# zipnn/zipnn

Hardware: NVIDIA H100
Metric: compress+decompress GB/s on bf16 tensors (higher is better)
Workload: dtype u8

## Files before the change

### zipnn_b200/csrc/decode.cuh

```cuda
#pragma once
#include <cuda.h>
#include "common.cuh"

#ifndef ZB_CPASYNC_L2
#define ZB_CPASYNC_L2 ".L2::128B"
#endif

#ifndef ZB_SIDE_SLOTS
#ifndef ZB_FUSED_MIN_BLOCKS
#define ZB_FUSED_MIN_BLOCKS 16
#endif
#define ZB_SIDE_SLOTS 4
#endif

namespace zb {

struct ItemTable;

enum : uint32_t { kModePlain = 0, kModeFused = 1, kModeGeneral = 2, kModeSkip = 3, kModeOverflow = 4 };
constexpr uint32_t kOverflowCtas = 32;
constexpr uint32_t kFillBytes = 64;

struct DecodeCfg {
  const uint8_t* body;
  uint8_t* out;
  uint64_t body_len;
  int G;
  uint64_t K;
  uint32_t chunk;
  uint64_t orig;
  int bits_mode;
  Ctrl* ctrl;
  ItemDesc* items;
  uint8_t* mode;
  uint32_t* slot;
  uint32_t* rlist;
  uint8_t* fill;
  uint8_t* planes;
  uint64_t pstride;
  uint32_t max_slots;
  uint32_t ovf_slots;
  uint32_t* olist;
  uint32_t* hlist;
  struct ItemTable* tables;
  uint32_t tma_flags;
  uint64_t k_full;
  uint64_t side_pred[3];
  uint32_t side_r0[3];
  uint64_t box_base, box_rows, box_pitch, box_len;
  uint64_t box_step_rows, box_step_cols;
  uint32_t box_fast;
  uint64_t c0;
};

constexpr uint32_t kBoxStep = 4096;

__device__ __forceinline__ bool box_meets(const DecodeCfg& cfg, uint64_t a, uint64_t n) {
  const uint64_t e0 = cfg.box_base + cfg.box_len;
  const uint64_t r = a < e0 ? 0 : (a - e0) / cfg.box_pitch + 1;
  return r < cfg.box_rows && cfg.box_base + r * cfg.box_pitch < a + n;
}
struct BoxCursor {
  int64_t row;
  uint64_t col;
};
__device__ __forceinline__ BoxCursor box_cursor(const DecodeCfg& cfg, uint64_t v) {
  BoxCursor k;
  if (v >= cfg.box_base) {
    const uint64_t q = (v - cfg.box_base) / cfg.box_pitch;
    k.row = (int64_t)q;
    k.col = v - cfg.box_base - q * cfg.box_pitch;
  } else {
    const uint64_t d = cfg.box_base - v, q = (d + cfg.box_pitch - 1) / cfg.box_pitch;
    k.row = -(int64_t)q;
    k.col = q * cfg.box_pitch - d;
  }
  return k;
}
__device__ __forceinline__ void box_advance(const DecodeCfg& cfg, BoxCursor& k) {
  k.row += (int64_t)cfg.box_step_rows;
  k.col += cfg.box_step_cols;
  if (k.col >= cfg.box_pitch) {
    k.col -= cfg.box_pitch;
    k.row++;
  }
}
__device__ __forceinline__ void box_store16(const DecodeCfg& cfg, uint8_t* __restrict__ out, const BoxCursor& k, const uint32_t (&r)[4]) {
  if (cfg.box_fast) {
    if (k.row >= 0 && (uint64_t)k.row < cfg.box_rows && k.col < cfg.box_len)
      *reinterpret_cast<uint4*>(out + (uint64_t)k.row * cfg.box_len + k.col) = make_uint4(r[0], r[1], r[2], r[3]);
    return;
  }
  int64_t row = k.row;
  uint64_t col = k.col;
#pragma unroll
  for (int i = 0; i < 16; i++) {
    if (row >= 0 && (uint64_t)row < cfg.box_rows && col < cfg.box_len) out[(uint64_t)row * cfg.box_len + col] = (uint8_t)(r[i >> 2] >> (8 * (i & 3)));
    if (++col == cfg.box_pitch) {
// ... 594 lines not shown
  bool active = false;
  uint64_t c = 0;
  int g = 0;
  if (item < nitems) {
    g = (int)(item / cfg.K);
    c = item - (uint64_t)g * cfg.K;
    if (cfg.mode[c] == kModeGeneral) {
      d = cfg.items[item];
      active = (d.kind == kHuf);
    }
  }
  if (__ballot_sync(0xffffffffu, active) == 0) return;
  planar_decode_item(S, cfg, d, active, slot, stream, active ? cfg.planes + ((uint64_t)cfg.slot[c] * cfg.G + g) * cfg.pstride : nullptr);
}

struct alignas(64) TmaMaps {
  CUtensorMap out;
  CUtensorMap side[3];
};
enum : uint32_t { kTmaOut = 1u, kTmaSide = 2u };

__device__ __forceinline__ void mbar_init(uint32_t bar_s, uint32_t count) {
  asm volatile("mbarrier.init.shared::cta.b64 [%0], %1;" ::"r"(bar_s), "r"(count) : "memory");
}
__device__ __forceinline__ void mbar_expect_tx(uint32_t bar_s, uint32_t bytes) {
  asm volatile("mbarrier.arrive.expect_tx.shared::cta.b64 _, [%0], %1;" ::"r"(bar_s), "r"(bytes) : "memory");
}
__device__ __forceinline__ void mbar_wait(uint32_t bar_s, uint32_t parity) {
  asm volatile(
      "{\n.reg .pred p;\nW_%=:\nmbarrier.try_wait.parity.shared::cta.b64 p, [%0], %1;\n@p bra D_%=;\nbra W_%=;\nD_%=:\n}\n" ::"r"(bar_s), "r"(parity)
      : "memory");
}
__device__ __forceinline__ void tma_load_2d(uint32_t dst_s, const CUtensorMap* map, uint32_t x, uint32_t y, uint32_t bar_s) {
  asm volatile("cp.async.bulk.tensor.2d.shared::cluster.global.mbarrier::complete_tx::bytes [%0], [%1, {%2, %3}], [%4];" ::"r"(dst_s),
               "l"((uint64_t)(uintptr_t)map), "r"(x), "r"(y), "r"(bar_s)
               : "memory");
}
__device__ __forceinline__ void tma_store_2d(const CUtensorMap* map, uint32_t src_s, uint32_t x, uint32_t y) {
  asm volatile("cp.async.bulk.tensor.2d.global.shared::cta.bulk_group [%0, {%2, %3}], [%1];" ::"l"((uint64_t)(uintptr_t)map), "r"(src_s), "r"(x), "r"(y)
               : "memory");
  asm volatile("cp.async.bulk.commit_group;" ::: "memory");
}
__device__ __forceinline__ void tma_store_wait_read() { asm volatile("cp.async.bulk.wait_group.read 0;" ::: "memory"); }
__device__ __forceinline__ void tma_store_wait_all() { asm volatile("cp.async.bulk.wait_group 0;" ::: "memory"); }
__device__ __forceinline__ void fence_proxy_async() { asm volatile("fence.proxy.async.shared::cta;" ::: "memory"); }

template <int G>
struct FusedGeom {
  static constexpr int kIters = 8 / G;
  static constexpr int NS = (G > 1) ? G - 1 : 1;
  static constexpr uint32_t kSlotBytes = 512u * ZB_SIDE_SLOTS;
  static constexpr int kTileIters = 2;
  static constexpr uint32_t kTileRow = 16u * kTileIters + 16u, kTileBytes = 32u * kTileRow;
  static constexpr uint32_t kTileRegion = (G == 2) ? 2u * kTileBytes : 0u;
  static constexpr uint32_t kSlotRegion = (G == 1) ? 0u : (uint32_t)(G - 1) * kSlotBytes;
  static constexpr uint32_t kSideAll = kSlotRegion > kTileRegion ? kSlotRegion : kTileRegion;
};
__host__ __device__ constexpr uint32_t fused_tail_bytes(int pb) { return pb == 0 ? 4096u : 2048u; }
__host__ __device__ constexpr uint32_t fused_tail_cap(int pb) { return fused_tail_bytes(pb) / 2u; }
template <int G>
__host__ __device__ constexpr size_t fused_smem_bytes(int pb) {
  return (pb == 0 ? (size_t)4096 + 32 * kRingBytes : (size_t)3072 + 16 * kRingBytes) + FusedGeom<G>::kSideAll + fused_tail_bytes(pb) + 32 * 128 + 16;
}
struct FusedSmem {
  unsigned char* raw;
  uint32_t base_s;
  uint32_t table_off;
  uint32_t ring_lo_off, ring_hi_off;
  uint32_t tail_off, bar_off, stage_off, side_off;
  __device__ __forceinline__ uint16_t* tail() const { return reinterpret_cast<uint16_t*>(raw + tail_off); }
  __device__ __forceinline__ uint8_t* ring(int lane) const { return raw + (lane < 16 ? ring_lo_off : ring_hi_off) + kRingBytes * (uint32_t)(lane & 15); }
  __device__ __forceinline__ uint8_t* weights(int slot) const { return raw + (slot < 4 ? ring_lo_off : ring_hi_off) + 256u * (uint32_t)(slot & 3); }
  __device__ __forceinline__ uint8_t (*stage() const)[128] { return reinterpret_cast<uint8_t (*)[128]>(raw + stage_off); }
};
template <int G, int PB>
__device__ __forceinline__ FusedSmem fused_smem_carve(unsigned char* raw) {
  FusedSmem S;
  S.raw = raw;
  S.base_s = (uint32_t)__cvta_generic_to_shared(raw);
  asm volatile("" : "+r"(S.base_s));
  uint32_t at;
  if (PB == 0) {
    S.table_off = 0;
    at = 4096;
  } else {
    S.table_off = (2048u - (S.base_s & 2047u)) & 2047u;
    S.ring_lo_off = S.table_off ? 0u : 2048u;
    at = 3072;
  }
  S.tail_off = at;
  at += fused_tail_bytes(PB);
  if (PB == 0) {
    S.ring_lo_off = at;
    at += 16 * kRingBytes;
  }
  S.ring_hi_off = at;
  at += 16 * kRingBytes;
  S.stage_off = at;
  at += 32 * 128;
  S.side_off = at;
  S.bar_off = at + FusedGeom<G>::kSideAll;
  return S;
}
template <int G>
__device__ __forceinline__ uint32_t side_tile_s(const FusedSmem& S, uint32_t st) { return S.base_s + S.side_off + st * FusedGeom<G>::kTileBytes; }
template <int G>
__device__ __forceinline__ uint32_t side_slots_s(const FusedSmem& S, int g) { return S.base_s + S.side_off + (uint32_t)g * FusedGeom<G>::kSlotBytes; }
static_assert(sizeof(FseDecSmall) <= 512, "small tANS scratch must fit in 4 stage rows");

struct SidePlane {
  const uint4* blk;
  uint32_t shift;
  uint32_t step;
  uint4 a, b;
  uint32_t slots_s;
  uint32_t swz;
};

__device__ __forceinline__ uint4 lds_u128(uint32_t saddr) {
  uint4 v;
  asm volatile("ld.shared.v4.u32 {%0, %1, %2, %3}, [%4];" : "=r"(v.x), "=r"(v.y), "=r"(v.z), "=r"(v.w) : "r"(saddr));
  return v;
}
constexpr uint32_t kSideSlots = ZB_SIDE_SLOTS;
__device__ __forceinline__ uint32_t side_slot(const SidePlane& sp, uint32_t j) { return sp.slots_s + (((j & (kSideSlots - 1u)) ^ sp.swz) << 4); }

__device__ __forceinline__ uint4 ldg128(const uint4* p) { return __ldg(p); }
__device__ __forceinline__ void take16(const uint4& a, const uint4& b, uint32_t shift, uint32_t (&out)[4]) {
  const uint32_t w[8] = {a.x, a.y, a.z, a.w, b.x, b.y, b.z, b.w};
  const uint32_t bs = (shift & 3) * 8;
  uint32_t t[7];
#pragma unroll
  for (int i = 0; i < 7; i++) t[i] = __funnelshift_r(w[i], w[i + 1], bs);
  const bool s4 = shift & 4, s8 = shift & 8;
  uint32_t u[5];
#pragma unroll
  for (int i = 0; i < 5; i++) u[i] = s8 ? t[i + 2] : t[i];
#pragma unroll
  for (int i = 0; i < 4; i++) out[i] = s4 ? u[i + 1] : u[i];
}

template <int W>
__device__ __forceinline__ void take16_w(const uint4& a, const uint4& b, uint32_t bit_shift, uint32_t (&out)[4]) {
  const uint32_t w[8] = {a.x, a.y, a.z, a.w, b.x, b.y, b.z, b.w};
#pragma unroll
  for (int i = 0; i < 4; i++) out[i] = __funnelshift_r(w[i + W], w[i + W + 1], bit_shift);
}

__device__ __forceinline__ uint32_t bitselect(uint32_t a, uint32_t b, uint32_t m) {
  uint32_t d;
  asm("lop3.b32 %0, %1, %2, %3, 0xE4;" : "=r"(d) : "r"(a), "r"(b), "r"(m));
  return d;
}
__device__ __forceinline__ void unrotate_planes_pre(uint32_t& lo, uint32_t& hi, uint32_t m) {
  const uint32_t sm = lo, e = hi;
  hi = bitselect(sm, e, m);
  lo = bitselect(e, sm, m);
}

__device__ __forceinline__ uint4* stage_unit(uint8_t (*stage)[128], int row, int unit) {
  return reinterpret_cast<uint4*>(&stage[row][((unit ^ row) & 7) * 16]);
}

template <int G>
__device__ __forceinline__ void emit_elements(uint32_t (&pl)[G][4], uint32_t rot_mask, uint8_t (*stage)[128], int lane, int unit0) {
  if (G == 1) {
    *stage_unit(stage, lane, unit0) = make_uint4(pl[0][0], pl[0][1], pl[0][2], pl[0][3]);
    return;
  }
#pragma unroll
  for (int q = 0; q < 4; q++) unrotate_planes_pre(pl[(G - 2) % G][q], pl[G - 1][q], rot_mask);
  uint32_t w[4 * G];
  if (G == 2) {
#pragma unroll
    for (int q = 0; q < 4; q++) {
      w[2 * q] = __byte_perm(pl[0][q], pl[1 % G][q], 0x5140);
      w[2 * q + 1] = __byte_perm(pl[0][q], pl[1 % G][q], 0x7362);
    }
  } else {
#pragma unroll
    for (int q = 0; q < 4; q++) {
      const uint32_t t0 = __byte_perm(pl[0][q], pl[1 % G][q], 0x5140), t1 = __byte_perm(pl[2 % G][q], pl[3 % G][q], 0x5140);
      const uint32_t t2 = __byte_perm(pl[0][q], pl[1 % G][q], 0x7362), t3 = __byte_perm(pl[2 % G][q], pl[3 % G][q], 0x7362);
      w[4 * q] = __byte_perm(t0, t1, 0x5410);
      w[4 * q + 1] = __byte_perm(t0, t1, 0x7632);
      w[4 * q + 2] = __byte_perm(t2, t3, 0x5410);
      w[4 * q + 3] = __byte_perm(t2, t3, 0x7632);
    }
  }
#pragma unroll
  for (int q = 0; q < G; q++) *stage_unit(stage, lane, unit0 + q) = make_uint4(w[4 * q], w[4 * q + 1], w[4 * q + 2], w[4 * q + 3]);
}

template <int G, class LUT>
__device__ __forceinline__ void fused_iteration(BitWindow& b, const LUT& lut, SidePlane (&side)[(G > 1) ? G - 1 : 1],
                                                const uint4* hi_block, bool guard, bool rot, uint8_t (*stage)[128], int lane, int unit0, uint32_t it,
                                                bool wait_store) {
  if (G > 1) {
#pragma unroll
    for (int g = 0; g < G - 1; g++) {
      const uint4* nb = side[g].blk + 3 * side[g].step;
      if (guard && side[g].step && nb > hi_block) nb = hi_block;
      cp_async16_s(side_slot(side[g], it + 3u), nb);
    }
  }
  uint32_t pl[G][4];
  decode16(b, lut, pl[G - 1]);
  if (wait_store) {
    if (lane == 0) tma_store_wait_read();
    __syncwarp();
  }
  if (G > 1) {
#pragma unroll
    for (int g = 0; g < G - 1; g++) take16(side[g].a, side[g].b, side[g].shift, pl[g]);
  }
  emit_elements<G>(pl, rot ? 0x80808080u : 0u, stage, lane, unit0);
  if (G > 1) {
#pragma unroll
    for (int g = 0; g < G - 1; g++) {
      side[g].a = side[g].b;
      side[g].b = lds_u128(side_slot(side[g], it + 2u));
      side[g].blk += side[g].step;
    }
  }
}

template <int G, int PB>
__global__ void __launch_bounds__(32, G == 4 ? 12 : ZB_FUSED_MIN_BLOCKS) k_huf_decode_fused(DecodeCfg cfg, uint8_t* __restrict__ out, const __grid_constant__ TmaMaps maps) {
  extern __shared__ __align__(1024) unsigned char smem_raw[];
  using Geo = FusedGeom<G>;
  using LUT = typename std::conditional<PB == 0, LutTwo, LutCol<(PB ? PB : 5)>>::type;
  constexpr int kIters = Geo::kIters;
  constexpr int NS = Geo::NS;
  const FusedSmem S = fused_smem_carve<G, PB>(smem_raw);
  const int lane = threadIdx.x, slot = lane >> 2, stream = lane & 3;
  const uint64_t K = cfg.K;
  const uint64_t ngroups = (K + kDecItemsPerWarp - 1) / kDecItemsPerWarp;
  if (PB != 0 && S.table_off > 1024u) {
    if (lane == 0 && blockIdx.x == 0) atomicOr(&cfg.ctrl->error, kErrUnsupported);
    return;
  }
  const uint32_t bar_s = S.base_s + S.bar_off;
  if (lane == 0) {
    mbar_init(bar_s, 1);
    mbar_init(bar_s + 8, 1);
    asm volatile("fence.mbarrier_init.release.cluster;" ::: "memory");
  }
  __syncwarp();
  uint32_t tiles_done = 0;
  bool store_pending = false;
  uint8_t (*const stage)[128] = S.stage();
  const uint32_t stage_s = S.base_s + S.stage_off;
  const bool rot = (cfg.bits_mode == 1) && (G > 1);
  const uint32_t rot_mask = rot ? 0x80808080u : 0u;
  const uint4* hi_block = reinterpret_cast<const uint4*>(((uintptr_t)(cfg.body + cfg.body_len) - 1) & ~(uintptr_t)15);

  for (uint64_t grp = blockIdx.x; grp < ngroups; grp += gridDim.x) {
    const uint64_t c = grp * kDecItemsPerWarp + slot;
    const bool active = (c < K) && cfg.mode[c] == kModeFused;
    if (__ballot_sync(0xffffffffu, active) == 0) continue;
    if (store_pending) {
      if (lane == 0) tma_store_wait_read();
      store_pending = false;
    }
    __syncwarp();

    ItemDesc d;
    d.kind = kRaw;
    d.src_off = 0;
    d.src_len = d.dec_len = 0;
    if (active) d = cfg.items[(uint64_t)(G - 1) * K + c];

    int lg = 0, hsize = -1, x_long = 0;
    uint32_t tail_at = 0;
    {
      uint8_t* weights = S.weights(slot);
      const bool builder = active && stream == 0;
      int nsym = 0;
      constexpr uint32_t kHdrSlot = 176;
      uint8_t* hdr = reinterpret_cast<uint8_t*>(S.tail()) + kHdrSlot * (uint32_t)slot;
      const uint8_t* tsrc = cfg.body + d.src_off;
      const uint32_t mis = (uint32_t)((uintptr_t)tsrc & 15u);
      if (active) {
        const uint8_t* body_end = cfg.body + cfg.body_len;
#pragma unroll
        for (int q = 0; q < 3; q++) {
          const int blk = stream + 4 * q;
          const uint8_t* g = tsrc - mis + 16 * blk;
          if (blk < (int)(kHdrSlot / 16) && g < body_end) *reinterpret_cast<uint4*>(hdr + 16 * blk) = ldg128(reinterpret_cast<const uint4*>(g));
        }
      }
      __syncwarp();
      if (builder) {
        FseDecSmall& D = *reinterpret_cast<FseDecSmall*>(&stage[4 * slot][0]);
        const uint32_t avail = kHdrSlot - mis;
        hsize = huf_read_weights(weights, &nsym, &lg, hdr + mis, d.src_len < avail ? d.src_len : avail, D);
        if (hsize >= 0) {
          x_long = PB == 0 ? lut2_tail_size(weights, nsym, lg) : lut_tail_size(weights, nsym, lg, PB, reinterpret_cast<uint16_t*>(&stage[4 * slot][0]));
          if (x_long < 0) hsize = -1;
        }
      }
      {
        const uint32_t mine = (builder && hsize >= 0) ? (uint32_t)x_long : 0u;
        uint32_t run = mine;
#pragma unroll
        for (int o = 4; o < 32; o <<= 1) {
          const uint32_t v = __shfl_up_sync(0xffffffffu, run, o);
          if (lane >= o) run += v;
        }
        tail_at = run - mine;
// ... 15 lines not shown
        nsym = __shfl_sync(0xffffffffu, nsym, lane & ~3);
        if (active && hsize >= 0)
          fill_lut_col<(PB ? PB : 5)>(reinterpret_cast<uint16_t*>(S.raw + S.table_off) + lane, S.tail() + tail_at, stream == 0, weights, nsym, lg, rot, (uint32_t)x_long,
                                      reinterpret_cast<const uint16_t*>(&stage[4 * slot][0]));
      }
      __syncwarp();
    }
    bool live = active && hsize >= 0;

    const uint8_t* p = cfg.body + d.src_off + (live ? hsize : 0);
    const uint32_t rest = live ? d.src_len - (uint32_t)hsize : 0;
    uint32_t l0 = 0, l1 = 0, l2 = 0, l3 = 0;
    if (live) {
      bool ok = rest >= 10;
      if (ok) {
        l0 = p[0] | (p[1] << 8);
        l1 = p[2] | (p[3] << 8);
        l2 = p[4] | (p[5] << 8);
        ok = l0 + l1 + l2 + 6 <= rest;
        l3 = rest - (l0 + l1 + l2 + 6);
        ok = ok && l0 && l1 && l2 && l3;
      }
      if (!ok) {
        atomicOr(&cfg.ctrl->error, kErrCorrupt);
        live = false;
      }
    }
    const uint32_t seg = d.dec_len >> 2;
    uint32_t s_off = 6, s_len = l0;
    if (stream == 1) { s_off += l0; s_len = l1; }
    if (stream == 2) { s_off += l0 + l1; s_len = l2; }
    if (stream == 3) { s_off += l0 + l1 + l2; s_len = l3; }
    const uint32_t out_off = (uint32_t)stream * seg;

    LUT lut;
    if constexpr (PB == 0) {
      lut.prim_s = S.base_s + S.table_off + 512u * (uint32_t)slot;
    } else {
      lut.col_s = S.base_s + S.table_off + 2u * (uint32_t)lane;
    }
    lut.tail_s = S.base_s + S.tail_off + 2u * tail_at;
    lut.hi_mask = 0x7FFu & ~((uint32_t)x_long - 1u);

    bool regular = live && c < cfg.k_full;
    if (G > 1 && regular) {
#pragma unroll
      for (int g = 0; g < G - 1; g++) {
        const ItemDesc t = cfg.items[(uint64_t)g * K + c];
        regular = regular && t.kind == kRaw && t.src_off == cfg.side_pred[g] + c * (uint64_t)(cfg.chunk / (uint32_t)G);
      }
    }
    regular = __all_sync(0xffffffffu, regular);
    const bool out_tma = regular && (cfg.tma_flags & kTmaOut);
    const bool side_tma = (G == 2) && regular && (cfg.tma_flags & kTmaSide);

    BitWindow b;
    if (live && !window_init(b, p + s_off, s_len, cfg.body, S.ring(lane))) {
      atomicOr(&cfg.ctrl->error, kErrCorrupt);
      live = false;
    }
    if (regular && !live) {
      b.cont = 0; b.s = 53; b.qm = 0; b.next = 0; b.fetch48 = 0; b.floor64 = 0xffffffffu; b.start_bit = 0;
      b.ring = S.ring(lane);
      b.ring_s = (uint32_t)__cvta_generic_to_shared(b.ring);
      b.gsrc = cfg.body;
    }

    const uint32_t rows_full = (seg >> 4) / kIters;
    if constexpr (G == 2) {
      if (side_tma) {
        const uint32_t y0 = (uint32_t)(grp * 32u);
        constexpr int kTI = Geo::kTileIters;
        constexpr int kTilesPerRow = kIters / kTI;
        const uint32_t ntiles = rows_full * (uint32_t)kTilesPerRow;
        const uint32_t r0 = cfg.side_r0[0];
        auto issue_tile = [&](uint32_t t) {
          const uint32_t st = (tiles_done + t) & 1u;
          mbar_expect_tx(bar_s + 8u * st, Geo::kTileBytes);
          tma_load_2d(side_tile_s<G>(S, st), &maps.side[0], 16u * (uint32_t)kTI * t, y0, bar_s + 8u * st);
        };
        if (lane == 0 && ntiles) issue_tile(0);
        uint8_t* flush_ptr = out + (grp * (uint64_t)kDecItemsPerWarp) * (uint64_t)cfg.chunk + (uint64_t)((uint32_t)(lane >> 3) * seg) * G +
                             (uint32_t)(lane & 7) * 16u;
        const uint32_t chunk_b = cfg.chunk;
        const bool chunk_256k = chunk_b == 262144u;
        const uint32_t bit_shift = (r0 & 3u) * 8u;
        auto run_rows = [&](auto wtag) {
          constexpr int W = decltype(wtag)::value;
          for (uint32_t row = 0; row < rows_full; row++) {
#pragma unroll
            for (int tr = 0; tr < kTilesPerRow; tr++) {
              const uint32_t t = row * (uint32_t)kTilesPerRow + (uint32_t)tr;
              const uint32_t n = tiles_done + t;
              __syncwarp();
              if (lane == 0 && t + 1 < ntiles) issue_tile(t + 1);
              mbar_wait(bar_s + 8u * (n & 1u), (n >> 1) & 1u);
              const uint32_t my_row = side_tile_s<G>(S, n & 1u) + (uint32_t)lane * Geo::kTileRow;
              uint4 blk[kTI + 1];
#pragma unroll
              for (int q = 0; q <= kTI; q++) blk[q] = lds_u128(my_row + 16u * (uint32_t)q);
#pragma unroll
              for (int ki = 0; ki < kTI; ki++) {
                uint32_t pl[G][4];
                decode16(b, lut, pl[G - 1]);
                take16_w<W>(blk[ki], blk[ki + 1], bit_shift, pl[0]);
                emit_elements<G>(pl, rot_mask, stage, lane, (tr * kTI + ki) * G);
              }
            }
            __syncwarp();
            if (chunk_256k) {
#pragma unroll
              for (int r = 0; r < 8; r++) *reinterpret_cast<uint4*>(flush_ptr + (size_t)r * 262144u) = *stage_unit(stage, r * 4 + (lane >> 3), lane & 7);
            } else {
#pragma unroll
              for (int r = 0; r < 8; r++) *reinterpret_cast<uint4*>(flush_ptr + (size_t)r * chunk_b) = *stage_unit(stage, r * 4 + (lane >> 3), lane & 7);
            }
            flush_ptr += 128;
            __syncwarp();
          }
        };
        switch (r0 >> 2) {
          case 0: run_rows(std::integral_constant<int, 0>{}); break;
          case 1: run_rows(std::integral_constant<int, 1>{}); break;
          case 2: run_rows(std::integral_constant<int, 2>{}); break;
          default: run_rows(std::integral_constant<int, 3>{}); break;
        }
        tiles_done += ntiles;
        if (live && !window_exact(b)) atomicOr(&cfg.ctrl->error, kErrCorrupt);
        continue;
      }
    }
    SidePlane side[NS];
    if (G > 1 && live) {
#pragma unroll
      for (int g = 0; g < G - 1; g++) {
        const uint64_t i = (uint64_t)g * K + c;
        const ItemDesc t = cfg.items[i];
        const uint8_t* q;
        if (t.kind == kRle) {
          q = cfg.fill + i * kFillBytes;
          side[g].step = 0;
        } else {
          q = cfg.body + t.src_off + out_off;
          side[g].step = 1;
        }
        side[g].shift = (uint32_t)((uintptr_t)q & 15);
        side[g].blk = reinterpret_cast<const uint4*>((uintptr_t)q & ~(uintptr_t)15);
        side[g].a = ldg128(side[g].blk);
        const uint4* nb = side[g].blk + side[g].step;
        side[g].b = ldg128((side[g].step && nb > hi_block) ? hi_block : nb);
        nb += side[g].step;
        side[g].swz = kSideSlots == 2 ? (((uint32_t)lane >> 2) & 1u) : (((uint32_t)lane >> 1) & 3u);
        side[g].slots_s = side_slots_s<G>(S, g) + 16u * kSideSlots * (uint32_t)lane;
        cp_async16_s(side_slot(side[g], 2u), (side[g].step && nb > hi_block) ? hi_block : nb);
      }
      cp_async_commit();
      cp_async_wait<0>();
    }

    const uint32_t my_rows = live ? rows_full : 0;
    uint32_t max_rows = my_rows;
#pragma unroll
    for (int o = 16; o; o >>= 1) max_rows = max(max_rows, __shfl_xor_sync(0xffffffffu, max_rows, o));
    if (out_tma) {
      const uint32_t y0 = (uint32_t)(grp * 32u);
      for (uint32_t row = 0; row < max_rows; row++) {
        const bool guard = row + 2 >= my_rows;
#pragma unroll
        for (int k = 0; k < kIters; k++)
          fused_iteration<G, LUT>(b, lut, side, hi_block, guard, rot, stage, lane, k * G, row * (uint32_t)kIters + (uint32_t)k, k == 0 && store_pending);
// ... 250 lines not shown
```

### zipnn_b200/csrc/common.cuh

```cuda
#pragma once
#include <cuda_runtime.h>
#include <stdint.h>
#include "huf_serial.cuh"

namespace zb {

struct Ctrl {
  uint32_t error;
  uint32_t overflow_count;
  uint64_t base[4];
  uint64_t total_len;
  uint64_t group_total[4];
  uint32_t work_counter;
  uint32_t regroup_count;
  uint32_t huf_count;
};
static_assert(sizeof(Ctrl) <= 256, "ctrl block");
constexpr size_t kCtrlBytes = 256;

struct ItemDesc {
  uint64_t src_off;
  uint32_t src_len;
  uint32_t dec_len;
  uint32_t kind;
  uint32_t pad;
};
enum : uint32_t { kRaw = 0, kRle = 1, kHuf = 2 };

enum : uint32_t { kErrCorrupt = 1u, kErrUnsupported = 2u, kErrWorkspace = 4u };

__host__ __device__ __forceinline__ uint32_t rot16(uint32_t u) {
  return ((u >> 8) & 0x00800080u) | ((u << 1) & 0xFF00FF00u) | (u & 0x007F007Fu);
}
__host__ __device__ __forceinline__ uint32_t unrot16(uint32_t u) {
  return ((u << 8) & 0x80008000u) | ((u >> 1) & 0x7F807F80u) | (u & 0x007F007Fu);
}
__host__ __device__ __forceinline__ uint32_t rot32(uint32_t u) {
  return ((u >> 8) & 0x00800000u) | ((u << 1) & 0xFF000000u) | (u & 0x007FFFFFu);
}
__host__ __device__ __forceinline__ uint32_t unrot32(uint32_t u) {
  return ((u << 8) & 0x80000000u) | ((u >> 1) & 0x7F800000u) | (u & 0x007FFFFFu);
}
template <int G>
__host__ __device__ __forceinline__ uint32_t rot_word(uint32_t u) {
  return G == 2 ? rot16(u) : (G == 4 ? rot32(u) : u);
}
template <int G>
__host__ __device__ __forceinline__ uint32_t unrot_word(uint32_t u) {
  return G == 2 ? unrot16(u) : (G == 4 ? unrot32(u) : u);
}

__host__ __device__ __forceinline__ uint32_t plane_len(uint32_t chunk_len, int G, int g) {
  return chunk_len / (uint32_t)G + ((uint32_t)g < chunk_len % (uint32_t)G ? 1u : 0u);
}

__device__ __forceinline__ uint32_t batch_find(const uint64_t* start, uint32_t n, uint64_t w) {
  uint32_t lo = 0, hi = n;
  while (hi - lo > 1) {
    const uint32_t mid = (lo + hi) >> 1;
    if (start[mid] <= w) lo = mid; else hi = mid;
  }
  return lo;
}

__device__ __forceinline__ uint64_t ld_u64_bytes(const uint8_t* p) {
  uint64_t v = 0;
#pragma unroll
  for (int i = 0; i < 8; i++) v |= (uint64_t)p[i] << (8 * i);
// ... 23 lines not shown
```

### zipnn_b200/csrc/zipnn_b200.cu

```cuda
#include "../../include/zipnn_b200.h"

#include <cuda.h>
#include <cuda_runtime.h>
#include <atomic>
#include <cstdio>
#include <cstdlib>
#include <cstring>
#include <mutex>
#include <numeric>
#include <vector>

#include "common.cuh"
#include "decode.cuh"
#include "decode_sync.cuh"
#include "encode.cuh"
#include "stage1.cuh"

using namespace zb;

namespace {

std::atomic<int> g_last_cuda_error{0};
std::atomic<unsigned long long> g_launches{0};

// ... 47 lines not shown
      a = take_event();
      cudaEventRecord(a, st);
    }
  }
  ~ScopedTimer() {
    if (a) {
      std::lock_guard<std::mutex> lk(g_timing_mu);
      cudaEvent_t b = take_event();
      cudaEventRecord(b, st);
      g_spans.push_back({id, a, b});
    }
  }
};

int sm_count_cached() {
  static int cached = 0;
  if (cached == 0) {
    int dev = 0, n = 0;
    if (cudaGetDevice(&dev) == cudaSuccess &&
        cudaDeviceGetAttribute(&n, cudaDevAttrMultiProcessorCount, dev) == cudaSuccess && n > 0)
      cached = n;
    else
      return 132;
  }
  return cached;
}

typedef CUresult (*EncodeTiledFn)(CUtensorMap*, CUtensorMapDataType, cuuint32_t, void*, const cuuint64_t*, const cuuint64_t*,
                                  const cuuint32_t*, const cuuint32_t*, CUtensorMapInterleave, CUtensorMapSwizzle,
                                  CUtensorMapL2promotion, CUtensorMapFloatOOBfill);
EncodeTiledFn tensor_map_encoder() {
  static EncodeTiledFn fn = [] {
    void* p = nullptr;
    cudaDriverEntryPointQueryResult q;
    if (cudaGetDriverEntryPoint("cuTensorMapEncodeTiled", &p, cudaEnableDefault, &q) != cudaSuccess || q != cudaDriverEntryPointSuccess) p = nullptr;
    (void)cudaGetLastError();
    return (EncodeTiledFn)p;
  }();
  return fn;
}
bool byte_map_2d(CUtensorMap* m, const void* base, uint64_t inner, uint64_t rows, uint64_t pitch, uint32_t box_inner, CUtensorMapSwizzle sw,
                 CUtensorMapL2promotion l2) {
  EncodeTiledFn enc = tensor_map_encoder();
  if (!enc || ((uintptr_t)base & 15) || (pitch & 15) || inner == 0 || rows == 0 || inner > 0xffffffffull || rows > 0xffffffffull) return false;
  cuuint64_t dims[2] = {inner, rows};
  cuuint64_t strides[1] = {pitch};
  cuuint32_t box[2] = {box_inner, 32};
  cuuint32_t es[2] = {1, 1};
  return enc(m, CU_TENSOR_MAP_DATA_TYPE_UINT8, 2, const_cast<void*>(base), dims, strides, box, es, CU_TENSOR_MAP_INTERLEAVE_NONE, sw, l2,
             CU_TENSOR_MAP_FLOAT_OOB_FILL_NONE) == CUDA_SUCCESS;
}

struct Knobs {
  int tma = 2, grid_mode = 1, warps_per_sm = 0;
  long long sync_max = -1;
  long long slice_piece = -1;
  size_t smem_pad = 0;
};
Knobs knobs() {
  Knobs k;
  if (const char* e = getenv("ZIPNN_B200_SLICE_PIECE_CHUNKS")) k.slice_piece = atoll(e);
  if (const char* e = getenv("ZIPNN_B200_TMA")) k.tma = atoi(e);
  if (const char* e = getenv("ZIPNN_B200_GRID_MODE")) k.grid_mode = atoi(e);
  if (const char* e = getenv("ZIPNN_B200_WARPS_PER_SM")) k.warps_per_sm = atoi(e);
  if (const char* e = getenv("ZIPNN_B200_SMEM_PAD")) k.smem_pad = (size_t)atoi(e);
  if (const char* e = getenv("ZIPNN_B200_SYNC_MAX")) k.sync_max = atoll(e);
  return k;
}

template <typename Kernel>
int resident_blocks(Kernel k, size_t smem) {
  int nb = 0;
  if (cudaOccupancyMaxActiveBlocksPerMultiprocessor(&nb, k, 32, smem) != cudaSuccess || nb < 1) nb = 1;
  return nb;
}

inline bool valid_layout(int num_buf, int bytes_mode, size_t chunk) {
  if (!(num_buf == 1 || num_buf == 2 || num_buf == 4)) return false;
  if (num_buf == 4 ? bytes_mode != 220 : bytes_mode != 10) return false;
  if (chunk == 0 || (chunk & (chunk - 1)) != 0 || chunk > (1ull << 31)) return false;
  if (chunk % (size_t)num_buf) return false;
  return true;
}

inline size_t round_up(size_t v, size_t a) { return (v + a - 1) / a * a; }
inline uint64_t num_chunks(size_t n, size_t chunk) { return (n + chunk - 1) / chunk; }

constexpr uint64_t kDefaultSlots = 64;
constexpr uint64_t kSyncTablesMaxChunks = 16384;
constexpr uint64_t kSyncDefaultMaxChunks = 3072;
struct DecWs {
  size_t items_off, mode_off, slot_off, rlist_off, olist_off, hlist_off, tables_off, fill_off, planes_off, pstride, fixed;
};
inline DecWs dec_ws_layout(size_t orig, int G, size_t chunk, uint64_t table_chunks = UINT64_MAX) {
  DecWs L;
  const uint64_t K = num_chunks(orig, chunk);
  if (table_chunks == UINT64_MAX) table_chunks = K <= kSyncTablesMaxChunks ? K : 0;
  L.items_off = kCtrlBytes;
  L.mode_off = round_up(L.items_off + sizeof(ItemDesc) * (size_t)G * K, 256);
  L.slot_off = round_up(L.mode_off + K, 256);
  L.rlist_off = round_up(L.slot_off + 4 * K, 256);
  L.olist_off = round_up(L.rlist_off + 4 * K, 256);
  L.hlist_off = round_up(L.olist_off + 4 * K, 256);
  L.tables_off = round_up(L.hlist_off + 4 * (size_t)G * K, 256);
  L.fill_off = round_up(L.tables_off + sizeof(ItemTable) * (size_t)G * table_chunks, 256);
  L.planes_off = round_up(L.fill_off + (size_t)kFillBytes * G * K, 256);
  L.pstride = round_up(chunk / (size_t)G, 16) + 16;
  L.fixed = L.planes_off + 256;
  return L;
}

template <typename F>
int dispatch_G(int G, F&& f) {
  switch (G) {
    case 1: return f(std::integral_constant<int, 1>());
    case 2: return f(std::integral_constant<int, 2>());
    default: return f(std::integral_constant<int, 4>());
  }
}

int read_ctrl_error(void* d_ws, cudaStream_t st) {
  uint32_t err = 0;
  ZB_CUDA(cudaMemcpyAsync(&err, d_ws, sizeof(uint32_t), cudaMemcpyDeviceToHost, st));
  ZB_CUDA(cudaStreamSynchronize(st));
  if (err & kErrCorrupt) return ZIPNN_B200_E_CORRUPT;
  if (err & kErrUnsupported) return ZIPNN_B200_E_UNSUPPORTED;
  if (err & kErrWorkspace) return ZIPNN_B200_E_CAPACITY;
// ... 160 lines not shown
      }
      static const int nb = [] {
        int v = 0;
        if (cudaOccupancyMaxActiveBlocksPerMultiprocessor(&v, k_huf_decode_sync<GG>, kSyncThreads, kSyncSmemBytes) != cudaSuccess || v < 1) v = 1;
        return v;
      }();
      const unsigned grid = (unsigned)std::min<uint64_t>(4 * nitems, (uint64_t)nb * sm_count_cached());
      {
        ScopedTimer tp(kKParseTables, st);
        k_parse_tables<<<(unsigned)((nitems + kParseWarps - 1) / kParseWarps), kParseWarps * 32, 0, st>>>(cfg);
        ZB_LAUNCHED();
      }
      ScopedTimer tm(kKHufDecodeSync, st);
      k_huf_decode_sync<GG><<<grid, kSyncThreads, kSyncSmemBytes, st>>>(cfg, (uint8_t*)d_out);
      ZB_LAUNCHED();
      return ZIPNN_B200_OK;
    });
    if (rc) return rc;
  } else {
    {
      const uint64_t groups = (K + kDecItemsPerWarp - 1) / kDecItemsPerWarp;
      if (groups > 0x7fffffffull) return ZIPNN_B200_E_ARG;
      const bool short_codes = (G >= 2 && bits_mode == 1);
      TmaMaps maps;
      memset(&maps, 0, sizeof(maps));
      cfg.tma_flags = 0;
      cfg.k_full = orig / chunk;
      const uint64_t last_len = orig - cfg.k_full * chunk;
      uint64_t at = 9ull * G * K;
      for (int g = 0; g < 3; g++) {
        cfg.side_pred[g] = at;
        cfg.side_r0[g] = (uint32_t)(((uintptr_t)d_body + at) & 15);
        if (g < G) at += cfg.k_full * (chunk / G) + plane_len((uint32_t)last_len, G, g);
      }
      if (cfg.k_full >= (uint64_t)kDecItemsPerWarp && chunk >= 2048 && (chunk / 4) * 4 == chunk) {
        if (byte_map_2d(&maps.out, d_out, chunk / 4, 4 * cfg.k_full, chunk / 4, 128, CU_TENSOR_MAP_SWIZZLE_128B, CU_TENSOR_MAP_L2_PROMOTION_NONE)) {
          cfg.tma_flags |= kTmaOut;
        if (G == 2) {
          const uint64_t seg = chunk / G / 4;
          const uint8_t* base = (const uint8_t*)d_body + cfg.side_pred[0] - cfg.side_r0[0];
          if (seg >= 64 && body_len >= cfg.side_pred[0] + 4 * cfg.k_full * seg &&
              byte_map_2d(&maps.side[0], base, seg + 16, 4 * cfg.k_full, seg, FusedGeom<2>::kTileRow, CU_TENSOR_MAP_SWIZZLE_NONE,
                          CU_TENSOR_MAP_L2_PROMOTION_L2_128B))
            cfg.tma_flags |= kTmaSide;
        }
        }
      }
      cfg.tma_flags &= (uint32_t)kn.tma;
      if (getenv("ZIPNN_B200_DEBUG")) fprintf(stderr, "[zipnn_b200] fused decode: K=%llu k_full=%llu tma_flags=%u side_r0=%u encoder=%p\n", (unsigned long long)K,
                                              (unsigned long long)cfg.k_full, cfg.tma_flags, cfg.side_r0[0], (void*)tensor_map_encoder());
      ScopedTimer tm(kKHufDecode, st);
      int rc = dispatch_G(G, [&](auto g) -> int {
        constexpr int GG = decltype(g)::value;
        const int sms = sm_count_cached();
        auto grid_for = [&](int nb) -> unsigned {
          if (kn.grid_mode == 1) return (unsigned)groups;
          if (kn.warps_per_sm > 0) nb = std::min(nb, kn.warps_per_sm);
          return (unsigned)std::min<uint64_t>(groups, (uint64_t)nb * sms);
        };
        if (short_codes) {
          const size_t smem = fused_smem_bytes<GG>(5) + kn.smem_pad;
          const int nb = resident_blocks(k_huf_decode_fused<GG, 5>, smem);
          k_huf_decode_fused<GG, 5><<<grid_for(nb), 32, smem, st>>>(cfg, (uint8_t*)d_out, maps);
        } else {
          const size_t smem = fused_smem_bytes<GG>(0) + kn.smem_pad;
          const int nb = resident_blocks(k_huf_decode_fused<GG, 0>, smem);
          k_huf_decode_fused<GG, 0><<<grid_for(nb), 32, smem, st>>>(cfg, (uint8_t*)d_out, maps);
        }
        ZB_LAUNCHED();
        return ZIPNN_B200_OK;
      });
      if (rc) return rc;
    }
    {
      const uint64_t warps = (nitems + kDecItemsPerWarp - 1) / kDecItemsPerWarp;
      if (warps > 0x7fffffffull) return ZIPNN_B200_E_ARG;
      ScopedTimer tm(kKHufDecodePlanar, st);
      k_huf_decode_planar<<<(unsigned)warps, 32, sizeof(DecodeSmem), st>>>(cfg);
      ZB_LAUNCHED();
    }
  }
  {
    const uint32_t tiles_per_chunk = (uint32_t)((chunk + kMergeTile - 1) / kMergeTile);
    const uint64_t ntiles = K * tiles_per_chunk;
    const int blocks = (int)std::min<uint64_t>(ntiles, (uint64_t)sm_count_cached() * 16);
    ScopedTimer tm(kKRegroup, st);
    int rc = dispatch_G(G, [&](auto g) -> int {
      k_regroup<decltype(g)::value><<<blocks, kMergeThreads, 0, st>>>(cfg, (uint8_t*)d_out);
      ZB_LAUNCHED();
      return ZIPNN_B200_OK;
    });
    if (rc) return rc;
  }
  if (cfg.ovf_slots) {
    ScopedTimer tm(kKDecodeOverflow, st);
    int rc = dispatch_G(G, [&](auto g) -> int {
      k_decode_overflow<decltype(g)::value><<<cfg.ovf_slots, kMergeThreads, sizeof(DecodeSmem), st>>>(cfg, (uint8_t*)d_out);
      ZB_LAUNCHED();
      return ZIPNN_B200_OK;
    });
    if (rc) return rc;
  }
  if (check) return read_ctrl_error(d_ws, st);
  return ZIPNN_B200_OK;
}

static size_t batch_header_bytes(int n) {
  return round_up(256 + sizeof(DecodeCfg) * (size_t)n + 3 * sizeof(uint64_t) * ((size_t)n + 1), 256);
}
static size_t batch_slice_bytes(const zipnn_b200_batch_item& it) {
  size_t w = 0;
  if (it.orig == 0) return 0;
  zipnn_b200_decompress_workspace_size(it.orig, it.num_buf, it.chunk, &w);
  return round_up(w, 256);
}

int zipnn_b200_decompress_batch_workspace_size(const zipnn_b200_batch_item* items, int n, size_t* out) {
  if (!out || n < 0 || (n && !items)) return ZIPNN_B200_E_ARG;
  size_t total = batch_header_bytes(n);
  for (int i = 0; i < n; i++) {
    if (!valid_layout(items[i].num_buf, items[i].bytes_mode, items[i].chunk)) return ZIPNN_B200_E_ARG;
// ... 305 lines not shown
```

Before: 429.6.

## Widen G=2 side-TMA staging rows to 256B and triple-buffer tile loads

For G==2 with nonzero PB, the side-plane TMA path now stages 256-byte rows per lane instead of 128, so each flush writes longer contiguous runs to global memory, and it uses three mbarrier-tracked tile stages instead of two, keeping two loads in flight. Shared memory sizing, barrier init and the stage swizzle are generalised to handle the wider rows. The side-TMA path is now gated on chunk divisibility by the wider row. The cost is more shared memory per block and a lower min-blocks launch bound (11), which may reduce occupancy.

Result: faster. 436.2 (median of 6 runs) (+1.5%).

```diff
diff --git a/zipnn_b200/csrc/decode.cuh b/zipnn_b200/csrc/decode.cuh
--- a/zipnn_b200/csrc/decode.cuh
+++ b/zipnn_b200/csrc/decode.cuh
@@ -744,16 +744,25 @@
   static constexpr uint32_t kSlotBytes = 512u * ZB_SIDE_SLOTS;
   static constexpr int kTileIters = 2;
   static constexpr uint32_t kTileRow = 16u * kTileIters + 16u, kTileBytes = 32u * kTileRow;
-  static constexpr uint32_t kTileRegion = (G == 2) ? 2u * kTileBytes : 0u;
   static constexpr uint32_t kSlotRegion = (G == 1) ? 0u : (uint32_t)(G - 1) * kSlotBytes;
-  static constexpr uint32_t kSideAll = kSlotRegion > kTileRegion ? kSlotRegion : kTileRegion;
 };
 __host__ __device__ constexpr uint32_t fused_tail_bytes(int pb) { return pb == 0 ? 4096u : 2048u; }
 __host__ __device__ constexpr uint32_t fused_tail_cap(int pb) { return fused_tail_bytes(pb) / 2u; }
+__host__ __device__ constexpr uint32_t fused_stage_row(int G, int pb) { return (G == 2 && pb != 0) ? 256u : 128u; }
+__host__ __device__ constexpr uint32_t fused_tile_stages(int G, int pb) { return fused_stage_row(G, pb) == 256u ? 3u : 2u; }
+template <int G>
+__host__ __device__ constexpr uint32_t fused_side_bytes(int pb) {
+  return G == 2 && fused_tile_stages(G, pb) * FusedGeom<G>::kTileBytes > FusedGeom<G>::kSlotRegion ? fused_tile_stages(G, pb) * FusedGeom<G>::kTileBytes
+                                                                                                     : FusedGeom<G>::kSlotRegion;
+}
+__host__ __device__ constexpr uint32_t fused_bar_bytes(int G, int pb) { return (8u * fused_tile_stages(G, pb) + 15u) & ~15u; }
 template <int G>
 __host__ __device__ constexpr size_t fused_smem_bytes(int pb) {
-  return (pb == 0 ? (size_t)4096 + 32 * kRingBytes : (size_t)3072 + 16 * kRingBytes) + FusedGeom<G>::kSideAll + fused_tail_bytes(pb) + 32 * 128 + 16;
-}
+  return (pb == 0 ? (size_t)4096 + 32 * kRingBytes : (size_t)3072 + 16 * kRingBytes) + fused_side_bytes<G>(pb) + fused_tail_bytes(pb) +
+         32 * fused_stage_row(G, pb) + fused_bar_bytes(G, pb);
+}
+template <int G, int PB>
+__host__ __device__ constexpr int fused_min_warps() { return fused_stage_row(G, PB) == 256u ? 11 : G == 4 ? 12 : ZB_FUSED_MIN_BLOCKS; }
 struct FusedSmem {
   unsigned char* raw;
   uint32_t base_s;
@@ -764,6 +773,8 @@
   __device__ __forceinline__ uint8_t* ring(int lane) const { return raw + (lane < 16 ? ring_lo_off : ring_hi_off) + kRingBytes * (uint32_t)(lane & 15); }
   __device__ __forceinline__ uint8_t* weights(int slot) const { return raw + (slot < 4 ? ring_lo_off : ring_hi_off) + 256u * (uint32_t)(slot & 3); }
   __device__ __forceinline__ uint8_t (*stage() const)[128] { return reinterpret_cast<uint8_t (*)[128]>(raw + stage_off); }
+  template <uint32_t RB>
+  __device__ __forceinline__ uint8_t (*stage_rows() const)[RB] { return reinterpret_cast<uint8_t (*)[RB]>(raw + stage_off); }
 };
 template <int G, int PB>
 __device__ __forceinline__ FusedSmem fused_smem_carve(unsigned char* raw) {
@@ -789,9 +800,9 @@
   S.ring_hi_off = at;
   at += 16 * kRingBytes;
   S.stage_off = at;
-  at += 32 * 128;
+  at += 32 * fused_stage_row(G, PB);
   S.side_off = at;
-  S.bar_off = at + FusedGeom<G>::kSideAll;
+  S.bar_off = at + fused_side_bytes<G>(PB);
   return S;
 }
 template <int G>
@@ -850,12 +861,13 @@
   lo = bitselect(e, sm, m);
 }
 
-__device__ __forceinline__ uint4* stage_unit(uint8_t (*stage)[128], int row, int unit) {
-  return reinterpret_cast<uint4*>(&stage[row][((unit ^ row) & 7) * 16]);
-}
-
-template <int G>
-__device__ __forceinline__ void emit_elements(uint32_t (&pl)[G][4], uint32_t rot_mask, uint8_t (*stage)[128], int lane, int unit0) {
+template <uint32_t RB>
+__device__ __forceinline__ uint4* stage_unit(uint8_t (*stage)[RB], int row, int unit) {
+  return reinterpret_cast<uint4*>(&stage[row][((unit & ~7) | ((unit ^ row) & 7)) * 16]);
+}
+
+template <int G, uint32_t RB>
+__device__ __forceinline__ void emit_elements(uint32_t (&pl)[G][4], uint32_t rot_mask, uint8_t (*stage)[RB], int lane, int unit0) {
   if (G == 1) {
     *stage_unit(stage, lane, unit0) = make_uint4(pl[0][0], pl[0][1], pl[0][2], pl[0][3]);
     return;
@@ -906,7 +918,7 @@
 #pragma unroll
     for (int g = 0; g < G - 1; g++) take16(side[g].a, side[g].b, side[g].shift, pl[g]);
   }
-  emit_elements<G>(pl, rot ? 0x80808080u : 0u, stage, lane, unit0);
+  emit_elements<G, 128>(pl, rot ? 0x80808080u : 0u, stage, lane, unit0);
   if (G > 1) {
 #pragma unroll
     for (int g = 0; g < G - 1; g++) {
@@ -918,7 +930,7 @@
 }
 
 template <int G, int PB>
-__global__ void __launch_bounds__(32, G == 4 ? 12 : ZB_FUSED_MIN_BLOCKS) k_huf_decode_fused(DecodeCfg cfg, uint8_t* __restrict__ out, const __grid_constant__ TmaMaps maps) {
+__global__ void __launch_bounds__(32, (fused_min_warps<G, PB>())) k_huf_decode_fused(DecodeCfg cfg, uint8_t* __restrict__ out, const __grid_constant__ TmaMaps maps) {
   extern __shared__ __align__(1024) unsigned char smem_raw[];
   using Geo = FusedGeom<G>;
   using LUT = typename std::conditional<PB == 0, LutTwo, LutCol<(PB ? PB : 5)>>::type;
@@ -932,10 +944,11 @@
     if (lane == 0 && blockIdx.x == 0) atomicOr(&cfg.ctrl->error, kErrUnsupported);
     return;
   }
+  constexpr uint32_t kStages = fused_tile_stages(G, PB);
   const uint32_t bar_s = S.base_s + S.bar_off;
   if (lane == 0) {
-    mbar_init(bar_s, 1);
-    mbar_init(bar_s + 8, 1);
+#pragma unroll
+    for (uint32_t st = 0; st < kStages; st++) mbar_init(bar_s + 8u * st, 1);
     asm volatile("fence.mbarrier_init.release.cluster;" ::: "memory");
   }
   __syncwarp();
@@ -1069,7 +1082,8 @@
     }
     regular = __all_sync(0xffffffffu, regular);
     const bool out_tma = regular && (cfg.tma_flags & kTmaOut);
-    const bool side_tma = (G == 2) && regular && (cfg.tma_flags & kTmaSide);
+    constexpr uint32_t kSideRow = fused_stage_row(G, PB), kSideRowIters = kSideRow / (16u * G);
+    const bool side_tma = (G == 2) && regular && (cfg.tma_flags & kTmaSide) && (cfg.chunk / (4u * G)) % (16u * kSideRowIters) == 0;
 
     BitWindow b;
     if (live && !window_init(b, p + s_off, s_len, cfg.body, S.ring(lane))) {
@@ -1088,31 +1102,39 @@
       if (side_tma) {
         const uint32_t y0 = (uint32_t)(grp * 32u);
         constexpr int kTI = Geo::kTileIters;
-        constexpr int kTilesPerRow = kIters / kTI;
-        const uint32_t ntiles = rows_full * (uint32_t)kTilesPerRow;
+        constexpr int kTilesPerRow = (int)kSideRowIters / kTI;
+        const uint32_t side_rows = (seg >> 4) / kSideRowIters;
+        const uint32_t ntiles = side_rows * (uint32_t)kTilesPerRow;
         const uint32_t r0 = cfg.side_r0[0];
         auto issue_tile = [&](uint32_t t) {
-          const uint32_t st = (tiles_done + t) & 1u;
+          const uint32_t st = (tiles_done + t) % kStages;
           mbar_expect_tx(bar_s + 8u * st, Geo::kTileBytes);
           tma_load_2d(side_tile_s<G>(S, st), &maps.side[0], 16u * (uint32_t)kTI * t, y0, bar_s + 8u * st);
         };
-        if (lane == 0 && ntiles) issue_tile(0);
-        uint8_t* flush_ptr = out + (grp * (uint64_t)kDecItemsPerWarp) * (uint64_t)cfg.chunk + (uint64_t)((uint32_t)(lane >> 3) * seg) * G +
-                             (uint32_t)(lane & 7) * 16u;
-        const uint32_t chunk_b = cfg.chunk;
-        const bool chunk_256k = chunk_b == 262144u;
+        if (lane == 0) {
+#pragma unroll
+          for (uint32_t t = 0; t + 1 < kStages; t++)
+            if (t < ntiles) issue_tile(t);
+        }
+        uint8_t (*const srows)[kSideRow] = S.stage_rows<kSideRow>();
+        constexpr uint32_t kRunLanes = kSideRow / 16u, kRunsPerStore = 32u / kRunLanes, kStores = kSideRow / 16u;
+        uint8_t* flush_ptr = out + (grp * (uint64_t)kDecItemsPerWarp) * (uint64_t)cfg.chunk + (uint64_t)((uint32_t)lane / kRunLanes * seg) * G +
+                             ((uint32_t)lane % kRunLanes) * 16u;
+        const uint32_t store_step = kRunsPerStore * (cfg.chunk / 4u);
+        const bool chunk_256k = cfg.chunk == 262144u;
         const uint32_t bit_shift = (r0 & 3u) * 8u;
         auto run_rows = [&](auto wtag) {
           constexpr int W = decltype(wtag)::value;
-          for (uint32_t row = 0; row < rows_full; row++) {
+          for (uint32_t row = 0; row < side_rows; row++) {
 #pragma unroll
             for (int tr = 0; tr < kTilesPerRow; tr++) {
               const uint32_t t = row * (uint32_t)kTilesPerRow + (uint32_t)tr;
               const uint32_t n = tiles_done + t;
               __syncwarp();
-              if (lane == 0 && t + 1 < ntiles) issue_tile(t + 1);
-              mbar_wait(bar_s + 8u * (n & 1u), (n >> 1) & 1u);
-              const uint32_t my_row = side_tile_s<G>(S, n & 1u) + (uint32_t)lane * Geo::kTileRow;
+              if (lane == 0 && t + kStages - 1 < ntiles) issue_tile(t + kStages - 1);
+              const uint32_t st = n % kStages;
+              mbar_wait(bar_s + 8u * st, (n / kStages) & 1u);
+              const uint32_t my_row = side_tile_s<G>(S, st) + (uint32_t)lane * Geo::kTileRow;
               uint4 blk[kTI + 1];
 #pragma unroll
               for (int q = 0; q <= kTI; q++) blk[q] = lds_u128(my_row + 16u * (uint32_t)q);
@@ -1121,18 +1143,21 @@
                 uint32_t pl[G][4];
                 decode16(b, lut, pl[G - 1]);
                 take16_w<W>(blk[ki], blk[ki + 1], bit_shift, pl[0]);
-                emit_elements<G>(pl, rot_mask, stage, lane, (tr * kTI + ki) * G);
+                emit_elements<G>(pl, rot_mask, srows, lane, (tr * kTI + ki) * G);
               }
             }
             __syncwarp();
+            const int src_row = (int)((uint32_t)lane / kRunLanes), unit = (int)((uint32_t)lane % kRunLanes);
             if (chunk_256k) {
 #pragma unroll
-              for (int r = 0; r < 8; r++) *reinterpret_cast<uint4*>(flush_ptr + (size_t)r * 262144u) = *stage_unit(stage, r * 4 + (lane >> 3), lane & 7);
+              for (uint32_t r = 0; r < kStores; r++)
+                *reinterpret_cast<uint4*>(flush_ptr + (size_t)r * (kRunsPerStore * 65536u)) = *stage_unit(srows, (int)(r * kRunsPerStore) + src_row, unit);
             } else {
 #pragma unroll
-              for (int r = 0; r < 8; r++) *reinterpret_cast<uint4*>(flush_ptr + (size_t)r * chunk_b) = *stage_unit(stage, r * 4 + (lane >> 3), lane & 7);
+              for (uint32_t r = 0; r < kStores; r++)
+                *reinterpret_cast<uint4*>(flush_ptr + (size_t)r * store_step) = *stage_unit(srows, (int)(r * kRunsPerStore) + src_row, unit);
             }
-            flush_ptr += 128;
+            flush_ptr += kSideRow;
             __syncwarp();
           }
         };
```

## Pack multiple decode warps per CTA with atomic work claiming in fused Huffman decode

Applied to the files above, without the earlier changes.

The fused Huffman decode kernel used to run one warp per CTA, with one CTA per group or a strided grid. It now packs several warps into a CTA, each with its own shared-memory region, and launches a persistent grid of about one CTA per SM. Warps pull work groups through an atomic counter, and the default is 13 or 10 warps for short-code bf16. This aims to cut CTA launch and scheduling overhead and to balance uneven per-group work. The costs are atomic contention, one large CTA per SM that can limit occupancy, and a reliance on the fused_next counter being zeroed before each launch.

Result: faster. 515.5 before, 536.5 after, median of 6 (+4.1%).

```diff
diff --git a/zipnn_b200/csrc/common.cuh b/zipnn_b200/csrc/common.cuh
--- a/zipnn_b200/csrc/common.cuh
+++ b/zipnn_b200/csrc/common.cuh
@@ -14,6 +14,7 @@
   uint32_t work_counter;
   uint32_t regroup_count;
   uint32_t huf_count;
+  uint32_t fused_next;
 };
 static_assert(sizeof(Ctrl) <= 256, "ctrl block");
 constexpr size_t kCtrlBytes = 256;
diff --git a/zipnn_b200/csrc/decode.cuh b/zipnn_b200/csrc/decode.cuh
--- a/zipnn_b200/csrc/decode.cuh
+++ b/zipnn_b200/csrc/decode.cuh
@@ -7,9 +7,6 @@
 #endif
 
 #ifndef ZB_SIDE_SLOTS
-#ifndef ZB_FUSED_MIN_BLOCKS
-#define ZB_FUSED_MIN_BLOCKS 16
-#endif
 #define ZB_SIDE_SLOTS 4
 #endif
 
@@ -44,6 +41,7 @@
   uint32_t* hlist;
   struct ItemTable* tables;
   uint32_t tma_flags;
+  uint32_t fused_claim;
   uint64_t k_full;
   uint64_t side_pred[3];
   uint32_t side_r0[3];
@@ -751,15 +749,37 @@
 __host__ __device__ constexpr uint32_t fused_tail_bytes(int pb) { return pb == 0 ? 4096u : 2048u; }
 __host__ __device__ constexpr uint32_t fused_tail_cap(int pb) { return fused_tail_bytes(pb) / 2u; }
 template <int G>
-__host__ __device__ constexpr size_t fused_smem_bytes(int pb) {
-  return (pb == 0 ? (size_t)4096 + 32 * kRingBytes : (size_t)3072 + 16 * kRingBytes) + FusedGeom<G>::kSideAll + fused_tail_bytes(pb) + 32 * 128 + 16;
-}
+__host__ __device__ constexpr uint32_t fused_warp_stride(int pb) {
+  return (pb == 0 ? 4096u + 32 * kRingBytes : 3072u + 16 * kRingBytes) + FusedGeom<G>::kSideAll + fused_tail_bytes(pb) + 32 * 128;
+}
+constexpr uint32_t kFusedBarBytes = 16;
+template <int G>
+__host__ __device__ constexpr size_t fused_smem_bytes(int pb, int warps = 1) {
+  return (size_t)warps * (fused_warp_stride<G>(pb) + kFusedBarBytes);
+}
+#ifndef ZB_FUSED_MAX_WARPS
+#define ZB_FUSED_MAX_WARPS 16
+#endif
+constexpr uint32_t kFusedCtaSmemMax = 232448;
+template <int G, int PB>
+__host__ __device__ constexpr int fused_smem_warps() {
+  return (int)(kFusedCtaSmemMax / (fused_warp_stride<G>(PB) + kFusedBarBytes));
+}
+template <int G, int PB>
+__host__ __device__ constexpr int fused_max_warps() {
+  return fused_smem_warps<G, PB>() < ZB_FUSED_MAX_WARPS ? fused_smem_warps<G, PB>() : ZB_FUSED_MAX_WARPS;
+}
+static_assert(fused_warp_stride<1>(0) % 1024 == 0 && fused_warp_stride<2>(0) % 1024 == 0 && fused_warp_stride<2>(5) % 1024 == 0 &&
+                  fused_warp_stride<4>(0) % 1024 == 0 && fused_warp_stride<4>(5) % 1024 == 0,
+              "every warp region must start on a 1 KiB boundary (fused_smem_carve)");
+static_assert(fused_smem_warps<2, 5>() == 17 && fused_smem_warps<4, 5>() == 14 && fused_smem_warps<2, 0>() == 13 && fused_smem_warps<1, 0>() == 16,
+              "the warps per CTA that DESIGN.md 3.1 lists");
 struct FusedSmem {
   unsigned char* raw;
   uint32_t base_s;
   uint32_t table_off;
   uint32_t ring_lo_off, ring_hi_off;
-  uint32_t tail_off, bar_off, stage_off, side_off;
+  uint32_t tail_off, stage_off, side_off;
   __device__ __forceinline__ uint16_t* tail() const { return reinterpret_cast<uint16_t*>(raw + tail_off); }
   __device__ __forceinline__ uint8_t* ring(int lane) const { return raw + (lane < 16 ? ring_lo_off : ring_hi_off) + kRingBytes * (uint32_t)(lane & 15); }
   __device__ __forceinline__ uint8_t* weights(int slot) const { return raw + (slot < 4 ? ring_lo_off : ring_hi_off) + 256u * (uint32_t)(slot & 3); }
@@ -791,7 +811,6 @@
   S.stage_off = at;
   at += 32 * 128;
   S.side_off = at;
-  S.bar_off = at + FusedGeom<G>::kSideAll;
   return S;
 }
 template <int G>
@@ -918,21 +937,23 @@
 }
 
 template <int G, int PB>
-__global__ void __launch_bounds__(32, G == 4 ? 12 : ZB_FUSED_MIN_BLOCKS) k_huf_decode_fused(DecodeCfg cfg, uint8_t* __restrict__ out, const __grid_constant__ TmaMaps maps) {
+__global__ void __launch_bounds__(32 * fused_max_warps<G, PB>(), 1) k_huf_decode_fused(DecodeCfg cfg, uint8_t* __restrict__ out, const __grid_constant__ TmaMaps maps) {
   extern __shared__ __align__(1024) unsigned char smem_raw[];
   using Geo = FusedGeom<G>;
   using LUT = typename std::conditional<PB == 0, LutTwo, LutCol<(PB ? PB : 5)>>::type;
   constexpr int kIters = Geo::kIters;
   constexpr int NS = Geo::NS;
-  const FusedSmem S = fused_smem_carve<G, PB>(smem_raw);
-  const int lane = threadIdx.x, slot = lane >> 2, stream = lane & 3;
+  constexpr uint32_t kStride = fused_warp_stride<G>(PB);
+  const uint32_t warp = threadIdx.x >> 5, nwarps = blockDim.x >> 5;
+  const FusedSmem S = fused_smem_carve<G, PB>(smem_raw + warp * kStride);
+  const int lane = threadIdx.x & 31, slot = lane >> 2, stream = lane & 3;
   const uint64_t K = cfg.K;
   const uint64_t ngroups = (K + kDecItemsPerWarp - 1) / kDecItemsPerWarp;
   if (PB != 0 && S.table_off > 1024u) {
     if (lane == 0 && blockIdx.x == 0) atomicOr(&cfg.ctrl->error, kErrUnsupported);
     return;
   }
-  const uint32_t bar_s = S.base_s + S.bar_off;
+  const uint32_t bar_s = S.base_s + (nwarps - warp) * kStride + kFusedBarBytes * warp;
   if (lane == 0) {
     mbar_init(bar_s, 1);
     mbar_init(bar_s + 8, 1);
@@ -947,7 +968,14 @@
   const uint32_t rot_mask = rot ? 0x80808080u : 0u;
   const uint4* hi_block = reinterpret_cast<const uint4*>(((uintptr_t)(cfg.body + cfg.body_len) - 1) & ~(uintptr_t)15);
 
-  for (uint64_t grp = blockIdx.x; grp < ngroups; grp += gridDim.x) {
+  const bool claim = cfg.fused_claim != 0;
+  auto next_group = [&](uint64_t after) -> uint64_t {
+    if (!claim) return after + (uint64_t)gridDim.x * nwarps;
+    uint32_t g = 0;
+    if (lane == 0) g = atomicAdd(&cfg.ctrl->fused_next, 1u);
+    return __shfl_sync(0xffffffffu, g, 0);
+  };
+  for (uint64_t grp = claim ? next_group(0) : (uint64_t)blockIdx.x * nwarps + warp; grp < ngroups; grp = next_group(grp)) {
     const uint64_t c = grp * kDecItemsPerWarp + slot;
     const bool active = (c < K) && cfg.mode[c] == kModeFused;
     if (__ballot_sync(0xffffffffu, active) == 0) continue;
diff --git a/zipnn_b200/csrc/zipnn_b200.cu b/zipnn_b200/csrc/zipnn_b200.cu
--- a/zipnn_b200/csrc/zipnn_b200.cu
+++ b/zipnn_b200/csrc/zipnn_b200.cu
@@ -123,7 +123,8 @@
 }
 
 struct Knobs {
-  int tma = 2, grid_mode = 1, warps_per_sm = 0;
+  int tma = 2;
+  int grid_mode = -1, warps_per_sm = 0;
   long long sync_max = -1;
   long long slice_piece = -1;
   size_t smem_pad = 0;
@@ -140,10 +141,67 @@
 }
 
 template <typename Kernel>
-int resident_blocks(Kernel k, size_t smem) {
+int resident_blocks(Kernel k, size_t smem, int threads = 32) {
   int nb = 0;
-  if (cudaOccupancyMaxActiveBlocksPerMultiprocessor(&nb, k, 32, smem) != cudaSuccess || nb < 1) nb = 1;
+  if (cudaOccupancyMaxActiveBlocksPerMultiprocessor(&nb, k, threads, smem) != cudaSuccess || nb < 1) nb = 1;
   return nb;
+}
+
+template <int G, int PB>
+int fused_cta_warps() {
+  static const int w = [] {
+    constexpr int wmax = fused_max_warps<G, PB>();
+    int best = 1;
+    if (cudaFuncSetAttribute(k_huf_decode_fused<G, PB>, cudaFuncAttributeMaxDynamicSharedMemorySize, (int)fused_smem_bytes<G>(PB, wmax)) == cudaSuccess) {
+      for (int v = wmax; v > 1; v--) {
+        int nb = 0;
+        if (cudaOccupancyMaxActiveBlocksPerMultiprocessor(&nb, k_huf_decode_fused<G, PB>, 32 * v, fused_smem_bytes<G>(PB, v)) == cudaSuccess && nb >= 1) {
+          best = v;
+          break;
+        }
+      }
+    }
+    (void)cudaGetLastError();
+    return best;
+  }();
+  return w;
+}
+
+template <int G, int PB>
+constexpr int fused_default_warps() {
+  return PB == 5 ? (G == 2 ? 13 : 10) : 0;
+}
+
+template <int G, int PB>
+void launch_fused(DecodeCfg cfg, uint8_t* out, const TmaMaps& maps, uint64_t groups, const Knobs& kn, cudaStream_t st) {
+  const uint64_t sms = (uint64_t)sm_count_cached();
+  constexpr int kDefault = fused_default_warps<G, PB>();
+  const int mode = kn.grid_mode >= 0 ? kn.grid_mode : (kDefault > 0 ? 2 : 1);
+  int W = 1;
+  unsigned grid;
+  size_t smem;
+  cfg.fused_claim = 0;
+  if (mode == 2) {
+    const int wmax = fused_cta_warps<G, PB>();
+    if (kn.warps_per_sm > 0) {
+      W = std::min(wmax, kn.warps_per_sm);
+    } else {
+      W = std::min(wmax, kDefault > 0 ? kDefault : wmax);
+      W = (int)std::min<uint64_t>((uint64_t)W, (groups + sms - 1) / sms);
+    }
+    grid = (unsigned)std::min<uint64_t>((groups + W - 1) / W, sms);
+    smem = fused_smem_bytes<G>(PB, W);
+    cfg.fused_claim = 1;
+  } else {
+    smem = fused_smem_bytes<G>(PB) + kn.smem_pad;
+    int nb = resident_blocks(k_huf_decode_fused<G, PB>, smem);
+    if (kn.warps_per_sm > 0) nb = std::min(nb, kn.warps_per_sm);
+    grid = mode == 1 ? (unsigned)groups : (unsigned)std::min<uint64_t>(groups, (uint64_t)nb * sms);
+  }
+  if (getenv("ZIPNN_B200_DEBUG"))
+    fprintf(stderr, "[zipnn_b200] fused launch: G=%d PB=%d mode=%d warps_per_cta=%d grid=%u resident_warps_per_sm=%d\n", G, PB, mode, W, grid,
+            W * resident_blocks(k_huf_decode_fused<G, PB>, smem, 32 * W));
+  k_huf_decode_fused<G, PB><<<grid, 32 * W, smem, st>>>(cfg, out, maps);
 }
 
 inline bool valid_layout(int num_buf, int bytes_mode, size_t chunk) {
@@ -410,21 +468,14 @@
       ScopedTimer tm(kKHufDecode, st);
       int rc = dispatch_G(G, [&](auto g) -> int {
         constexpr int GG = decltype(g)::value;
-        const int sms = sm_count_cached();
-        auto grid_for = [&](int nb) -> unsigned {
-          if (kn.grid_mode == 1) return (unsigned)groups;
-          if (kn.warps_per_sm > 0) nb = std::min(nb, kn.warps_per_sm);
-          return (unsigned)std::min<uint64_t>(groups, (uint64_t)nb * sms);
-        };
-        if (short_codes) {
-          const size_t smem = fused_smem_bytes<GG>(5) + kn.smem_pad;
-          const int nb = resident_blocks(k_huf_decode_fused<GG, 5>, smem);
-          k_huf_decode_fused<GG, 5><<<grid_for(nb), 32, smem, st>>>(cfg, (uint8_t*)d_out, maps);
-        } else {
-          const size_t smem = fused_smem_bytes<GG>(0) + kn.smem_pad;
-          const int nb = resident_blocks(k_huf_decode_fused<GG, 0>, smem);
-          k_huf_decode_fused<GG, 0><<<grid_for(nb), 32, smem, st>>>(cfg, (uint8_t*)d_out, maps);
+        if constexpr (GG > 1) {
+          if (short_codes) {
+            launch_fused<GG, 5>(cfg, (uint8_t*)d_out, maps, groups, kn, st);
+            ZB_LAUNCHED();
+            return ZIPNN_B200_OK;
+          }
         }
+        launch_fused<GG, 0>(cfg, (uint8_t*)d_out, maps, groups, kn, st);
         ZB_LAUNCHED();
         return ZIPNN_B200_OK;
       });
```
